# KumarRobotics/top_down_renderer

Hardware: AMD Instinct MI355X
Metric: particle-updates/sec (render+score+resample) (higher is better)
Workload: dtype f32

## Files before the change

include/tdr.h:

```cpp
#ifndef TDR_H_
#define TDR_H_

#include <stddef.h>
#include <stdint.h>

#ifdef __cplusplus
extern "C" {
#endif

#define TDR_OK 0
#define TDR_ERR_ARG (-1)
#define TDR_ERR_HIP (-2)
#define TDR_ERR_NOMEM (-3)

#define TDR_MAX_CLASSES 15
#define TDR_ST_FIELDS 7
enum { TDR_ST_INIT_X = 0, TDR_ST_INIT_Y = 1, TDR_ST_DX = 2, TDR_ST_DY = 3, TDR_ST_THETA = 4, TDR_ST_SCALE = 5,
       TDR_ST_HAVE_INIT = 6 };

typedef struct tdr_state {
  float init_x_px, init_y_px, dx_m, dy_m, theta, scale;
  uint8_t have_init;
  uint8_t pad_[3];
} tdr_state;
// ... 165 lines not shown
int tdr_config_compact(int on);
int tdr_config_shift_uniform(int mode);
float tdr_config_shift_uniform_span(float cells);
int tdr_config_ray_split(int k);
int tdr_config_cart_skip(int on);
int tdr_config_init_mfma(int on);
int tdr_config_uw_waves(int on);
int64_t tdr_shift_uniform_launches(void);

int tdr_profile_enable(int on);
int tdr_profile_score_ms(double* total_ms, int64_t* launches);
int tdr_profile_shares(double* dense_ms, double* scattered_ms, int64_t* scattered_particles);
int tdr_profile_variants(int64_t out[16]);

int64_t tdr_config_tuning(const char* name, int64_t value);
int tdr_selftest_score(void);
int tdr_k_selftest_round(const float* x, int64_t n, float limit, int32_t* out, void* stream);
int tdr_libm_variant(void);
int tdr_libm_force_variant(int variant);
int tdr_sincosf_host(const float* x, int64_t n, int variant, float* sin_out, float* cos_out);
int tdr_k_selftest_sincos(const float* x, int64_t n, float* sin_out, float* cos_out, void* stream);
int tdr_logf_host(const float* x, int64_t n, float* out);
int tdr_k_selftest_logf(const float* x, int64_t n, float* out, void* stream);
int tdr_k_selftest_atan2(const float* y, const float* x, int64_t n, float* out, void* stream);

int tdr_k_states_aos_to_soa(const tdr_state* aos, int64_t n, float* st, int64_t cap, void* stream);
int tdr_k_states_soa_to_aos(const float* st, int64_t cap, int64_t n, tdr_state* aos, void* stream);
size_t tdr_locality_tmp_ints(int64_t n, int map_rows, int map_cols);
int tdr_k_locality_order(const float* st, int64_t cap, int64_t n, int map_rows, int map_cols, int32_t* perm_out,
                         int32_t* keys_tmp, void* stream);
size_t tdr_locality_pose_tmp_ints(int64_t n);
int tdr_k_locality_order_pose(const float* st, int64_t cap, int64_t n, int map_rows, int map_cols, float theta_radius,
                              int32_t* perm_out, int32_t* keys_tmp, void* stream);

typedef struct tdr_map tdr_map;
typedef struct tdr_renderer tdr_renderer;
typedef struct tdr_filter tdr_filter;

int tdr_map_create(tdr_map** out);
void tdr_map_destroy(tdr_map* m);
int tdr_map_set(tdr_map* m, const float* class_maps, const uint8_t* class_mask, int ncls, int rows, int cols,
                float resolution, int center_x, int center_y);
int tdr_map_set_labels(tdr_map* m, const uint8_t* label_img, int img_h, int img_w, const int32_t* flatten_lut,
                       int lut_size, int ncls, float resolution, int center_x, int center_y);
int tdr_map_sample_pts_polar(tdr_map* m, int nb, int nr, float ang_res);
int tdr_map_polar_shape(const tdr_map* m, int* nb, int* nr);
int tdr_map_info(const tdr_map* m, int* ncls, int* rows, int* cols, float* resolution, int* have_map);
int tdr_map_center(const tdr_map* m, int* center_x, int* center_y);
int tdr_map_local_map(tdr_map* m, int polar, float cx, float cy, float scale_or_rot, float res, int rows, int cols,
                      float* dists_out, uint8_t* mask_out);
int tdr_map_classes_at_point(const tdr_map* m, int px, int py, uint32_t* class_bits);
int tdr_map_best_rel_pos(tdr_map* m, const float* preds, int K, float best_rel_pos[2], float* best_diff);
int tdr_map_local_geo_map(tdr_map* m, int polar, float cx, float cy, float scale_or_rot, float res, int rows, int cols,
                          float* dists_out);
int tdr_map_load_cache(tdr_map* m, const char* cache_dir, const char* map_path, int num_classes, float resolution,
                       int center_x, int center_y, int* loaded);
int tdr_map_save_cache(tdr_map* m, const char* cache_dir, const char* map_path);
int tdr_map_save_rasters(tdr_map* m, const char* dir);
int tdr_png_read_gray8_host(const char* path, uint8_t* px_out, int64_t capacity, int* w, int* h);
int tdr_png_write_gray8_host(const char* path, const uint8_t* px, int w, int h);
int tdr_map_load_rasters(tdr_map* m, const char* dir, int num_classes, float resolution, int center_x, int center_y);
#define TDR_SVG_NO_KEY 0xFFFFFFFFu
int tdr_svg_parse_host(const char* path, float size_out[2], int64_t* n_poly, int64_t* n_vert, uint32_t* keys_out,
                       int64_t* offsets_out, float* verts_out);
int tdr_map_load_polygons(tdr_map* m, const float* verts, const int64_t* poly_offsets, const int32_t* poly_class,
                          int64_t n_poly, int width, int height, int num_classes, const int32_t* exclusive, int n_excl,
// ... 79 lines not shown
```

top_down_renderer_amd/_lib.py:

```python
import ctypes as C
import os

_PKG = os.path.dirname(os.path.abspath(__file__))
SO_PATH = os.environ.get("TDR_LIB_PATH") or os.path.join(_PKG, "libtdr_hip.so")

TDR_ST_FIELDS = 7
TDR_MAX_CLASSES = 15
TDR_SVG_NO_KEY = 0xFFFFFFFF


class FilterParamsC(C.Structure):
    _fields_ = [
        ("pos_cov", C.c_float), ("theta_cov", C.c_float), ("regularization", C.c_float),
        ("init_pos_px_x", C.c_float), ("init_pos_px_y", C.c_float), ("init_pos_px_cov", C.c_float),
        ("init_pos_m_x", C.c_float), ("init_pos_m_y", C.c_float),
        ("init_pos_deg_theta", C.c_float), ("init_pos_deg_cov", C.c_float),
        ("force_on_map", C.c_int32),
        ("fixed_scale", C.c_float), ("scale_log_min", C.c_float), ("scale_log_max", C.c_float),
        ("num_classes", C.c_int32),
        ("class_weights", C.c_float * 16),
    ]


class MapDescC(C.Structure):
# ... 158 lines not shown
    "tdr_renderer_create": (_i, [_vp, C.POINTER(_vp)]),
    "tdr_renderer_destroy": (None, [_vp]),
    "tdr_renderer_render": (_i, [_vp, _i, _vp, _i, _i, _i64, _f, _f, _i, _i, _i, _vp]),
    "tdr_renderer_render_geo": (_i, [_vp, _i, _vp, _i, _i64, _i64, _f, _f, _i, _i, _vp]),
    "tdr_filter_create": (_i, [_vp, _i, C.POINTER(FilterParamsC), _u32, C.POINTER(_vp)]),
    "tdr_filter_destroy": (None, [_vp]),
    "tdr_filter_configure": (_i, [_vp, _i, _i]),
    "tdr_filter_initialize_particles": (_i, [_vp]),
    "tdr_filter_set_states": (_i, [_vp, _vp, _i64]),
    "tdr_filter_get_states": (_i, [_vp, _vp, _i64]),
    "tdr_filter_propagate": (_i, [_vp, _f, _f, _f]),
    "tdr_filter_update": (_i, [_vp, _vp, _vp, _f, _i64]),
    "tdr_filter_update_geo": (_i, [_vp, _vp, _vp, _f, _i64]),
    "tdr_filter_compute_weights": (_i, [_vp, _vp, _vp, _f]),
    "tdr_filter_get_raw_weights": (_i, [_vp, _vp, _i64]),
    "tdr_filter_get_last_dist": (_i, [_vp, _vp, _i64]),
    "tdr_filter_propagate_freeze": (_i, [_vp, _f, _f, _f, _i]),
    "tdr_filter_init_one": (_i, [_vp]),
    "tdr_filter_share_rng": (_i, [_vp, _vp]),
    "tdr_init_particle_host": (_i, [_vp, _vp, _i, _i, _i, _f, _vp, _vp]),
    "tdr_filter_get_weights": (_i, [_vp, _vp, _i64]),
    "tdr_filter_get_resample_indices": (_i, [_vp, _vp, _i64]),
    "tdr_filter_mean_cov": (_i, [_vp, _i, _vp, _vp]),
    "tdr_filter_freeze_scale": (_i, [_vp]),
    "tdr_filter_is_scale_frozen": (_i, [_vp]),
    "tdr_filter_scale": (_f, [_vp]),
    "tdr_filter_num_particles": (_i64, [_vp]),
    "tdr_filter_update_map": (_i, [_vp, _vp, _vp, _i, _i, _i, _f, _i, _i]),
    "tdr_set_error": (_i, [_i, C.c_char_p]),
    "tdr_locality_tmp_ints": (C.c_size_t, [_i64, _i, _i]),
    "tdr_locality_pose_tmp_ints": (C.c_size_t, [_i64]),
    "tdr_k_locality_order_pose": (_i, [_vp, _i64, _i64, _i, _i, _f, _vp, _vp, _vp]),
    "tdr_k_locality_order": (_i, [_vp, _i64, _i64, _i, _i, _vp, _vp, _vp]),
}

_lib = None


class TdrError(RuntimeError):
    pass


def load():
    global _lib
    if _lib is not None:
        return _lib
    if not os.path.exists(SO_PATH):
        raise TdrError(
            f"{SO_PATH} is missing: build the HIP extension first (python -m top_down_renderer_amd.build, or "
            "__graft_entry__.build()).  There is no CPU fallback.")
    L = C.CDLL(SO_PATH)
    for name, (res, args) in SIGNATURES.items():
        fn = getattr(L, name)
        fn.restype = res
        fn.argtypes = args
    _lib = L
    return L


def check(rc):
    if rc != 0:
        raise TdrError(f"libtdr_hip error {rc}: {load().tdr_last_error().decode()}")
```

top_down_renderer_amd/build.py:

```python
import os
import shutil
import subprocess
import sys
from concurrent.futures import ThreadPoolExecutor

PKG = os.path.dirname(os.path.abspath(__file__))
ROOT = os.path.dirname(PKG)
SRC = [os.path.join(PKG, "csrc", f) for f in
       ("tdr_core.hip", "tdr_map.hip", "tdr_raster.hip", "tdr_score.hip", "tdr_score_su.hip", "tdr_score_ray.hip", "tdr_score_cart.hip", "tdr_filter.hip", "tdr_rng.hip", "tdr_prefix.hip",
        "tdr_geo.hip", "tdr_cmap.hip", "tdr_active.hip", "tdr_poly.hip", "tdr_host.cpp", "tdr_comm.cpp", "tdr_gmm.cpp", "tdr_png.cpp",
        "tdr_svg.cpp")]
HDR = [os.path.join(ROOT, "include", "tdr.h")] + \
      [os.path.join(PKG, "csrc", f) for f in ("tdr_common.h", "tdr_sincosf.h", "tdr_atan2f.h", "tdr_score_su.h", "tdr_score_dev.h", "tdr_score_su_asm.h", "tdr_score_cart.h", "tdr_score_cart_asm.h", "tdr_logf.h", "tdr_mt_jump.h")]
OUT = os.path.join(PKG, "libtdr_hip.so")
OBJ_DIR = os.path.join(PKG, "_obj")
STAMP = os.path.join(PKG, "libtdr_hip.toolchain.txt")

CFLAGS = ["--offload-arch=gfx950", "-O3", "-std=c++17", "-ffp-contract=off", "-fPIC", "-I", os.path.join(ROOT, "include")]
LDFLAGS = ["--offload-arch=gfx950", "-shared", "-fPIC", "-ldl", "-lz"]
FILE_FLAGS = {"tdr_score.hip": ["-mllvm", "-amdgpu-mfma-vgpr-form"],
              "tdr_score_su.hip": ["-mllvm", "-structurizecfg-skip-uniform-regions"],
              "tdr_score_cart.hip": ["-mllvm", "-structurizecfg-skip-uniform-regions"]}


def hipcc():
    exe = shutil.which("hipcc") or "/opt/rocm/bin/hipcc"
    if not os.path.exists(exe):
        raise RuntimeError("hipcc not found: the HIP extension cannot be built (there is no CPU fallback)")
    return exe


def _obj(src):
    return os.path.join(OBJ_DIR, os.path.basename(src) + ".o")


def _stale(target, deps):
    if not os.path.exists(target):
        return True
    t = os.path.getmtime(target)
    return any(os.path.getmtime(d) > t for d in deps)


def needs_build():
    return _stale(OUT, SRC + HDR + [os.path.abspath(__file__)])


# ... 38 lines not shown
```

top_down_renderer_amd/csrc/tdr_filter.hip:

```cpp
#include <random>

#include <rocprim/device/device_radix_sort.hpp>
using TdrSortConfig = rocprim::radix_sort_config<rocprim::default_config, rocprim::merge_sort_config<512, 512, 4>, rocprim::default_config>;

#include "tdr_common.h"
#include "tdr_sincosf.h"

__device__ __forceinline__ uint32_t mulhi32(uint32_t a, uint32_t b) { return __umulhi(a, b); }
__device__ void philox4x32_10(uint32_t c[4], uint32_t k0, uint32_t k1) {
#pragma unroll
  for (int r = 0; r < 10; r++) {
    uint32_t hi0 = mulhi32(0xD2511F53u, c[0]), lo0 = 0xD2511F53u * c[0];
    uint32_t hi1 = mulhi32(0xCD9E8D57u, c[2]), lo1 = 0xCD9E8D57u * c[2];
    uint32_t n0 = hi1 ^ c[1] ^ k0, n1 = lo1, n2 = hi0 ^ c[3] ^ k1, n3 = lo0;
    c[0] = n0; c[1] = n1; c[2] = n2; c[3] = n3;
    k0 += 0x9E3779B9u; k1 += 0xBB67AE85u;
  }
}

__global__ void propagate_kernel(float* __restrict__ st, int64_t cap, int64_t n, float* __restrict__ last_dist,
                                 float tx, float ty, float omega, int scale_freeze, float pos_cov, float theta_cov,
                                 const float* __restrict__ z4, uint64_t seed, uint64_t step, int64_t index_base,
                                 int libm_fma) {
  const int64_t p = (int64_t)blockIdx.x * blockDim.x + threadIdx.x;
  if (p >= n) return;
  float z[4];
  if (z4) {
    z[0] = z4[4 * p]; z[1] = z4[4 * p + 1]; z[2] = z4[4 * p + 2]; z[3] = z4[4 * p + 3];
  } else {
    uint64_t gi = (uint64_t)(index_base + p);
    uint32_t c[4] = {(uint32_t)gi, (uint32_t)(gi >> 32), (uint32_t)step, (uint32_t)(step >> 32)};
    philox4x32_10(c, (uint32_t)seed, (uint32_t)(seed >> 32));
    float u0 = ((float)(c[0] >> 8) + 1.0f) * (1.0f / 16777216.0f), u1 = (float)(c[1] >> 8) * (1.0f / 16777216.0f);
    float u2 = ((float)(c[2] >> 8) + 1.0f) * (1.0f / 16777216.0f), u3 = (float)(c[3] >> 8) * (1.0f / 16777216.0f);
    float r0 = sqrtf(-2.0f * logf(u0)), r1 = sqrtf(-2.0f * logf(u2));
// ... 744 lines not shown
  s.dx_m = st[TDR_ST_DX * cap + p];
  s.dy_m = st[TDR_ST_DY * cap + p];
  s.theta = st[TDR_ST_THETA * cap + p];
  s.scale = st[TDR_ST_SCALE * cap + p];
  s.have_init = st[TDR_ST_HAVE_INIT * cap + p] != 0.f;
  s.pad_[0] = s.pad_[1] = s.pad_[2] = 0;
  aos[p] = s;
}
extern "C" int tdr_k_states_aos_to_soa(const tdr_state* aos, int64_t n, float* st, int64_t cap, void* stream) {
  if (!aos || !st || n < 0 || cap < n) return fail(TDR_ERR_ARG, "aos_to_soa: bad arguments");
  if (n == 0) return TDR_OK;
  hipLaunchKernelGGL(aos_to_soa_kernel, dim3((unsigned)cdiv(n, 256)), dim3(256), 0, (hipStream_t)stream, aos, n, st,
                     cap);
  LAUNCH_CHECK("aos_to_soa");
  return TDR_OK;
}
extern "C" int tdr_k_states_soa_to_aos(const float* st, int64_t cap, int64_t n, tdr_state* aos, void* stream) {
  if (!aos || !st || n < 0 || cap < n) return fail(TDR_ERR_ARG, "soa_to_aos: bad arguments");
  if (n == 0) return TDR_OK;
  hipLaunchKernelGGL(soa_to_aos_kernel, dim3((unsigned)cdiv(n, 256)), dim3(256), 0, (hipStream_t)stream, st, cap, n,
                     aos);
  LAUNCH_CHECK("soa_to_aos");
  return TDR_OK;
}

__device__ __forceinline__ uint32_t spread_bits16(uint32_t v) {
  v &= 0xFFFFu;
  v = (v | (v << 8)) & 0x00FF00FFu;
  v = (v | (v << 4)) & 0x0F0F0F0Fu;
  v = (v | (v << 2)) & 0x33333333u;
  v = (v | (v << 1)) & 0x55555555u;
  return v;
}
__global__ void loc_key_kernel(const float* __restrict__ st, int64_t cap, int64_t n, float xmax, float ymax,
                               uint32_t* __restrict__ keys, int32_t* __restrict__ vals) {
  const int64_t p = (int64_t)blockIdx.x * blockDim.x + threadIdx.x;
  if (p >= n) return;
  const float sc = st[TDR_ST_SCALE * cap + p];
  float cx = st[TDR_ST_DX * cap + p] * sc + st[TDR_ST_INIT_X * cap + p];
  float cy = st[TDR_ST_DY * cap + p] * sc + st[TDR_ST_INIT_Y * cap + p];
  if (!(cx == cx)) cx = 0.f;
  if (!(cy == cy)) cy = 0.f;
  const uint32_t hx = (uint32_t)fminf(fmaxf(cx * 2.f, 0.f), xmax);
  const uint32_t hy = (uint32_t)fminf(fmaxf(cy * 2.f, 0.f), ymax);
  keys[p] = spread_bits16(hx) | (spread_bits16(hy) << 1);
  vals[p] = (int32_t)p;
}

__device__ __forceinline__ uint64_t spread_bits21_3(uint64_t v) {
  v &= 0x1FFFFFull;
  v = (v | (v << 32)) & 0x1F00000000FFFFull;
  v = (v | (v << 16)) & 0x1F0000FF0000FFull;
  v = (v | (v << 8)) & 0x100F00F00F00F00Full;
  v = (v | (v << 4)) & 0x10C30C30C30C30C3ull;
  v = (v | (v << 2)) & 0x1249249249249249ull;
  return v;
}
__global__ void loc_key_pose_kernel(const float* __restrict__ st, int64_t cap, int64_t n, float xmax, float ymax,
                                    float theta_step, uint64_t* __restrict__ keys, int32_t* __restrict__ vals) {
  const int64_t p = (int64_t)blockIdx.x * blockDim.x + threadIdx.x;
  if (p >= n) return;
  const float sc = st[TDR_ST_SCALE * cap + p];
  float cx = st[TDR_ST_DX * cap + p] * sc + st[TDR_ST_INIT_X * cap + p];
  float cy = st[TDR_ST_DY * cap + p] * sc + st[TDR_ST_INIT_Y * cap + p];
  float th = st[TDR_ST_THETA * cap + p];
  if (!(cx == cx)) cx = 0.f;
  if (!(cy == cy)) cy = 0.f;
  if (!(fabsf(th) < 1e6f)) th = 0.f;
  th = th - 6.2831855f * floorf(th / 6.2831855f);
  const uint64_t hx = (uint64_t)fminf(fmaxf(cx * 2.f, 0.f), xmax);
  const uint64_t hy = (uint64_t)fminf(fmaxf(cy * 2.f, 0.f), ymax);
  const uint64_t ht = (uint64_t)fminf(fmaxf(th / theta_step, 0.f), 2097151.f);
  keys[p] = spread_bits21_3(hx) | (spread_bits21_3(hy) << 1) | (spread_bits21_3(ht) << 2);
  vals[p] = (int32_t)p;
}
static size_t radix_tmp_bytes64(int64_t n) {
  size_t bytes = 0;
  uint64_t* k = nullptr;
  int32_t* v = nullptr;
// ... 3 lines not shown
}
extern "C" size_t tdr_locality_pose_tmp_ints(int64_t n) {
  if (n < 1) n = 1;
  return (size_t)(5 * n + 64) + (radix_tmp_bytes64(n) + 3) / 4 + 64;
}
extern "C" int tdr_k_locality_order_pose(const float* st, int64_t cap, int64_t n, int map_rows, int map_cols,
                                         float theta_radius, int32_t* perm_out, int32_t* keys_tmp, void* stream) {
  if (!st || !perm_out || !keys_tmp || n < 0 || cap < n || map_rows < 1 || map_cols < 1 || !(theta_radius > 0.f))
    return fail(TDR_ERR_ARG, "locality_order_pose: bad arguments");
  if (map_rows > 1000000 || map_cols > 1000000) return fail(TDR_ERR_ARG, "locality_order_pose: map too large");
  if (n == 0) return TDR_OK;
  hipStream_t s = (hipStream_t)stream;
  uint64_t* keys_in = reinterpret_cast<uint64_t*>(keys_tmp);
  uint64_t* keys_out = keys_in + n;
  int32_t* vals_in = keys_tmp + 4 * n;
  void* tmp = keys_tmp + 5 * n + 64 - ((5 * n) % 64);
  size_t tmp_bytes = radix_tmp_bytes64(n);
  hipLaunchKernelGGL(loc_key_pose_kernel, dim3((unsigned)cdiv(n, 256)), dim3(256), 0, s, st, cap, n,
                     (float)(2 * map_cols - 1), (float)(2 * map_rows - 1), 0.5f / theta_radius, keys_in, vals_in);
  LAUNCH_CHECK("loc_key_pose");
  HIP_TRY(rocprim::radix_sort_pairs(tmp, tmp_bytes, keys_in, keys_out, vals_in, perm_out, (size_t)n, 0u, 63u, s, false));
  return TDR_OK;
}

static size_t radix_tmp_bytes(int64_t n) {
  size_t bytes = 0;
  uint32_t* k = nullptr;
  int32_t* v = nullptr;
  hipError_t e = rocprim::radix_sort_pairs<TdrSortConfig>(nullptr, bytes, k, k, v, v, (size_t)n, 0u, 32u, (hipStream_t)0, false);
  if (e != hipSuccess || bytes == 0) bytes = (size_t)(n + 4096) * 16;
  return bytes;
}

extern "C" size_t tdr_locality_tmp_ints(int64_t n, int map_rows, int map_cols) {
  (void)map_rows; (void)map_cols;
  if (n < 1) n = 1;
  return (size_t)(3 * n + 64) + (radix_tmp_bytes(n) + 3) / 4 + 64;
}

extern "C" int tdr_k_locality_order(const float* st, int64_t cap, int64_t n, int map_rows, int map_cols,
                                    int32_t* perm_out, int32_t* keys_tmp, void* stream) {
  if (!st || !perm_out || !keys_tmp || n < 0 || cap < n || map_rows < 1 || map_cols < 1)
    return fail(TDR_ERR_ARG, "locality_order: bad arguments");
  if (map_rows > 32767 || map_cols > 32767) return fail(TDR_ERR_ARG, "locality_order: map larger than 32767 px");
  if (n == 0) return TDR_OK;
  hipStream_t s = (hipStream_t)stream;
  uint32_t* keys_in = reinterpret_cast<uint32_t*>(keys_tmp);
  uint32_t* keys_out = keys_in + n;
  int32_t* vals_in = keys_tmp + 2 * n;
  void* tmp = keys_tmp + 3 * n + 64 - ((3 * n) % 64);
  size_t tmp_bytes = radix_tmp_bytes(n);
  hipLaunchKernelGGL(loc_key_kernel, dim3((unsigned)cdiv(n, 256)), dim3(256), 0, s, st, cap, n,
                     (float)(2 * map_cols - 1), (float)(2 * map_rows - 1), keys_in, vals_in);
  LAUNCH_CHECK("loc_key");
  unsigned bits = 2;
  while ((1u << (bits / 2)) < (unsigned)(2 * std::max(map_rows, map_cols)) && bits < 32) bits += 2;
  HIP_TRY(rocprim::radix_sort_pairs<TdrSortConfig>(tmp, tmp_bytes, keys_in, keys_out, vals_in, perm_out, (size_t)n, 0u, bits, s,
                                    false));
  return TDR_OK;
}
```

top_down_renderer_amd/csrc/tdr_score.hip:

```cpp
#include <type_traits>

#include "tdr_common.h"
#include "tdr_sincosf.h"

struct ScoreArgs {
  const float* rec;
  int rows, cols;
  float resolution;
  const float* tab;
  const float* utab;
  const float* scan_pk;
  int nb, nr;
  float res;
  const float* st;
  int64_t cap, n;
  const int32_t* order;
  const int32_t* count;
  const int32_t* slot_base;
  int use_theta_override;
  float theta_override;
  int only_uninit;
  int group, nchunks;
  int64_t npad;
  float* part;
// ... 1387 lines not shown
                                  float* __restrict__ st, int64_t cap) {
  const int64_t p = (int64_t)blockIdx.x * blockDim.x + threadIdx.x;
  if (p < n && res_flag[p] != 0.f) {
    st[TDR_ST_THETA * cap + p] = res_theta[p];
    st[TDR_ST_HAVE_INIT * cap + p] = 1.f;
  }
}
__global__ void init_fixup_kernel(const float* __restrict__ res_flag, int64_t n, float regularization,
                                  float* __restrict__ raw_w) {
  const int64_t p = (int64_t)blockIdx.x * blockDim.x + threadIdx.x;
  if (p < n && res_flag[p] == 2.f) raw_w[p] = (float)(1. / (double)(3.402823466e+38f + regularization));
}

static int g_init_mfma = 1;
static bool init_use_mfma() { return g_init_mfma != 0; }
extern "C" int tdr_config_init_mfma(int on) {
  if (on >= 0) g_init_mfma = on ? 1 : 0;
  return g_init_mfma;
}
#define TDR_CART_WAVE_MUL 2
static int64_t g_score_waves = 131072;
static int g_score_group = 0;
static int g_su_group = 0;
static int g_init_ahead = 1;
static int64_t score_wave_target() { return g_score_waves; }
extern "C" int tdr_config_prefix_head(int);
extern "C" int tdr_config_ray_block_major(int);
extern "C" int tdr_config_ray_patch(int);
extern "C" int tdr_config_ray_borrow(int);
extern "C" int tdr_config_cart_seg_rows(int);
extern "C" int tdr_config_mt_stretches(int);
extern "C" int tdr_config_su_wave_span(int);
extern "C" int tdr_config_su_lds_pad(int);
extern "C" int64_t tdr_config_tuning(const char* name, int64_t value) {
  if (!name) return -1;
  const std::string n(name);
  if (n == "score_waves") { if (value > 0) g_score_waves = value; return g_score_waves; }
  if (n == "score_group") { if (value >= 0) g_score_group = (int)value; return g_score_group; }
  if (n == "su_group") { if (value >= 0) g_su_group = (int)value; return g_su_group; }
  if (n == "init_ahead") { if (value >= 1) g_init_ahead = (int)std::min<int64_t>(value, 3); return g_init_ahead; }
  if (n == "prefix_head") return tdr_config_prefix_head((int)std::max<int64_t>(value, -1));
  if (n == "ray_borrow") return tdr_config_ray_borrow((int)std::max<int64_t>(value, -1));
  if (n == "ray_patch") return tdr_config_ray_patch((int)std::max<int64_t>(value, -1));
  if (n == "ray_block_major") return tdr_config_ray_block_major((int)std::max<int64_t>(value, -1));
  if (n == "cart_seg_rows") return tdr_config_cart_seg_rows((int)std::max<int64_t>(value, -1));
  if (n == "mt_stretches") return tdr_config_mt_stretches((int)std::max<int64_t>(value, -1));
  if (n == "su_lds_pad") return tdr_config_su_lds_pad((int)std::max<int64_t>(value, -1));
  if (n == "su_wave_span") return tdr_config_su_wave_span((int)std::max<int64_t>(value, -1));
  return -1;
}
static void choose_chunks(int64_t n, int nr, int& rpc, int& nchunks, int target_mul = 1) {
  int64_t nbatches = cdiv(std::max<int64_t>(n, 1), 64);
  int64_t want = std::max<int64_t>(1, cdiv(score_wave_target() * target_mul, nbatches));
  nchunks = (int)std::min<int64_t>(nr, want);
  rpc = (int)cdiv(nr, nchunks);
  nchunks = (int)cdiv(nr, rpc);
}

__global__ void utab_kernel(const float* __restrict__ tab, int64_t n2, float scale, float res,
                            float* __restrict__ utab) {
  const int64_t k = (int64_t)blockIdx.x * blockDim.x + threadIdx.x;
  if (k < n2) utab[k] = (tab[k] * scale) * res;
}

static int score_group_rings(int nb, int nr, int rf, int64_t n_total) {
  const int forced = g_score_group;
  const int64_t ring_bytes = std::max<int64_t>((int64_t)nb * rf * 4, 1);
  int g = (int)std::min<int64_t>(8, (32 * 1024) / ring_bytes);
  const int64_t chunks_wanted = cdiv(2048, cdiv(std::max<int64_t>(n_total, 1), 256));
  g = (int)std::min<int64_t>(g, std::max<int64_t>(1, nr / std::max<int64_t>(chunks_wanted, 1)));
  if (forced > 0) g = forced;
  g = std::max(1, std::min<int>(g, (int)((60 * 1024) / ring_bytes)));
  if (g >= TDR_SCORE_U) g -= g % TDR_SCORE_U;
  return std::max(g, 1);
}
extern "C" size_t tdr_map_rec16_bytes(int ncls, int rows, int cols) {
  if (ncls < 1 || ncls > 7 || rows < 1 || cols < 1) return 0;
  const uint64_t bytes = (uint64_t)(rows + 2) * (uint64_t)(cols + 2) * 32 + 32;
  if (bytes > 0xFFFFFFFFull || (uint64_t)(cols + 2) * 32 >= (1u << 24)) return 0;
  return (size_t)bytes;
}
// ... 733 lines not shown
```

top_down_renderer_amd/csrc/tdr_score_su.hip:

```cpp
#include <rocprim/device/device_radix_sort.hpp>

#include <atomic>

#include "tdr_score_dev.h"
#include "tdr_score_su.h"
#include "tdr_score_su_asm.h"

#define SU_CODE_FULL 0xFFu
#define SU_CODE_FULL_ALL 0xFEu
#define SU_CODE_PAD 0xFDu
#define SU_NSECT 8
#define SU_BOX_WORDS 4096

struct SuArgs {
  const uint32_t* crec;
  const uint32_t* kmask;
  int kcolw;
  unsigned kmask_off;
  const uint32_t* dict_int;
  int dict_n, ctiles_r;
  int pkcol;
  const int32_t* inexact;
  int rows, cols;
  float resolution;
  const float* tab_su;
  const uint32_t* desc;
  const float* bbox;
  const float* scan_pk;
  int nb, nr;
  float res;
  const float* st;
  int64_t cap;
  const int32_t* slots;
  const int32_t* nslots;
  int group, nchunks, ncls;
  int64_t npad;
  uint32_t* part;
// ... 768 lines not shown
    t->phase = 0;
    t->best_ms = 3.0e38f;
    t->round_best = t->best;
  }
  t->open = hipEventRecord(t->e0, s) == hipSuccess;
  t->trial_calls++;
  return kSpanCand[t->phase];
}
void tdr_su_span_end(SpanTuner* t, hipStream_t s) {
  if (g_su_span_fixed || !t || !t->open) return;
  t->open = false;
  t->pending = hipEventRecord(t->e1, s) == hipSuccess;
}
static float g_su_wave_span = 0.f;
extern "C" int tdr_config_su_wave_span(int cells) {
  if (cells >= 0) g_su_wave_span = (float)cells;
  return (int)g_su_wave_span;
}
float tdr_su_wave_span() { return g_su_wave_span; }
static int g_su_lds_pad = 0;
extern "C" int tdr_config_su_lds_pad(int bytes) {
  if (bytes >= 0) g_su_lds_pad = bytes;
  return g_su_lds_pad;
}
static std::atomic<int64_t> g_su_launches{0};
extern "C" int64_t tdr_shift_uniform_launches(void) { return g_su_launches.load(); }
bool tdr_su_shape_ok(int nb, int nr, int group, int64_t n_total) {
  if (g_su_mode == 0) return false;
  if (group % 4 != 0 || nb > 4095) return false;
  if (g_su_mode == 2) return true;
  if ((int64_t)nb * nr < 8192) return false;
  return n_total >= (int64_t)64 * nb;
}
static size_t su_sort_tmp_bytes(int64_t n) {
  size_t bytes = 0;
  uint32_t* k = nullptr;
  int32_t* v = nullptr;
  hipError_t e = rocprim::radix_sort_pairs(nullptr, bytes, k, k, v, v, (size_t)std::max<int64_t>(n, 1), 0u, 12u,
                                           (hipStream_t)0, false);
  if (e != hipSuccess || bytes == 0) bytes = (size_t)(n + 4096) * 16;
  return bytes;
}
SuWs tdr_su_ws(int nb, int nr, int group, int64_t n) {
  SuWs w;
  const int64_t nchunks = cdiv(nr, group), nbins = nchunks * nb * group;
  int64_t o = 0;
  auto take = [&](int64_t words) { const int64_t at = o; o += (words + 63) / 64 * 64; return at; };
  w.tab_su = take(2 * nbins);
  w.desc = take(4 * nbins);
  w.bbox = take(nchunks * SU_NSECT * 4);
  w.keys_in = take(n);
  w.keys_out = take(n);
  w.vals_in = take(n);
  w.vals_out = take(n);
  w.ints = take(3 * ((int64_t)nb + 1) + TDR_SU_TAIL_INTS);
  w.slots = take(su_npad(n, nb));
  w.slots2 = take(su_npad(n, nb));
  w.wave_tmp = take(2 * (su_npad(n, nb) / 64 + 1));
  w.sort_tmp = take((int64_t)((su_sort_tmp_bytes(n) + 3) / 4));
  const int64_t T = tdr_ray_padded_samples(nb, nr);
  w.ray_tab = take(2 * T);
  w.ray_desc = take((T + 1) / 2);
  w.ray_multi = take((int64_t)nb * nr);
  w.ray_rad = take(T / nb);
  w.total = o;
  return w;
}

int tdr_su_order(const SuLaunch& L, const SuWs& W, hipStream_t s, const int32_t** slots_out, const int32_t** counts_out) {
  int32_t* base = L.ws;
  uint32_t* keys_in = reinterpret_cast<uint32_t*>(base + W.keys_in);
  uint32_t* keys_out = reinterpret_cast<uint32_t*>(base + W.keys_out);
  int32_t* vals_in = base + W.vals_in;
  int32_t* vals_out = base + W.vals_out;
  int* cnt = base + W.ints;
  const int nkeys = L.nb + 1;
  int* start = cnt + nkeys;
  int* slot_start = start + nkeys;
  int* counts = slot_start + nkeys;
  int32_t* slots = base + W.slots;
  const int64_t n = L.n;
  HIP_TRY(hipMemsetAsync(cnt, 0, sizeof(int) * (size_t)(3 * nkeys + TDR_SU_TAIL_INTS), s));
  HIP_TRY(hipMemsetAsync(slots, 0xFF, sizeof(int32_t) * (size_t)L.npad, s));
  hipLaunchKernelGGL(su_key_kernel, dim3((unsigned)cdiv(n, 256)), dim3(256), sizeof(int) * (size_t)nkeys, s, L.st, L.cap, n,
                     L.perm, L.nb, L.span, keys_in, vals_in, cnt);
  LAUNCH_CHECK("su_key");
  hipLaunchKernelGGL(su_offsets_kernel, dim3(1), dim3(256), 0, s, (const int*)cnt, nkeys, start, slot_start, counts);
  LAUNCH_CHECK("su_offsets");
  unsigned bits = 1;
  while ((1u << bits) < (unsigned)nkeys) bits++;
  size_t tmp_bytes = su_sort_tmp_bytes(n);
  HIP_TRY(rocprim::radix_sort_pairs(base + W.sort_tmp, tmp_bytes, keys_in, keys_out, vals_in, vals_out, (size_t)n, 0u, bits,
                                    s, false));
  hipLaunchKernelGGL(su_scatter_kernel, dim3((unsigned)cdiv(n, 256)), dim3(256), 0, s, (const uint32_t*)keys_out,
                     (const int32_t*)vals_out, n, (const int*)start, (const int*)slot_start, slots);
  LAUNCH_CHECK("su_scatter");
  if (L.wave_span > 0.f && L.nb > 1) {
    int32_t* slots2 = base + W.slots2;
    int32_t* keep = base + W.wave_tmp;
    int32_t* moved = keep + (L.npad / 64 + 1);
    int32_t* old_counts = counts + 7;
    const int64_t nwaves = L.npad / 64;
    hipLaunchKernelGGL(su_wave_far_kernel, dim3((unsigned)cdiv(nwaves, 4)), dim3(256), 0, s, L.st, L.cap, (const int32_t*)slots,
                       (const int32_t*)counts, L.wave_span, keep, moved);
    hipLaunchKernelGGL(su_compact_offsets_kernel, dim3(1), dim3(256), 0, s, keep, moved, counts, old_counts);
    hipLaunchKernelGGL(su_compact_scatter_kernel, dim3((unsigned)cdiv(L.npad, 256)), dim3(256), 0, s, (const int32_t*)slots,
                       (const int32_t*)keep, (const int32_t*)moved, (const int32_t*)counts, (const int32_t*)old_counts, slots2);
    hipLaunchKernelGGL(su_copy_slots_kernel, dim3((unsigned)cdiv(L.npad, 256)), dim3(256), 0, s, (const int32_t*)slots2,
                       (const int32_t*)counts, slots);
    LAUNCH_CHECK("su_reroute");
  }
  *slots_out = slots;
  *counts_out = counts;
  return TDR_OK;
}
int tdr_su_prepare(const SuLaunch& L, const SuWs& W, hipStream_t s, const int32_t** slots_out, const int32_t** counts_out) {
  if (int rc = tdr_su_order(L, W, s, slots_out, counts_out)) return rc;
  int32_t* base = L.ws;
  float* tab_su = reinterpret_cast<float*>(base + W.tab_su);
  uint32_t* desc = reinterpret_cast<uint32_t*>(base + W.desc);
  const int64_t ndesc = (int64_t)L.nchunks * L.nb * L.group;
  const int lc = L.map->cwords == 1 ? 3 : (L.map->cwords == 2 ? 2 : 1);
  const int ckconst = ((L.map->rows >> lc) + 2) * 128 + 128;
  const unsigned plane_bytes = (unsigned)(tdr_cmap_plane_words(L.map->ncls, L.map->rows, L.map->cols) * 4);
  const unsigned pbase = (unsigned)(tdr_cmap_plane_offset_words(L.map->ncls, L.map->rows, L.map->cols) * 4) +
                         (unsigned)(plane_trows(L.map->rows) * 128) + 128u;
  hipLaunchKernelGGL(su_prep_kernel, dim3((unsigned)cdiv(ndesc, 256)), dim3(256), 0, s, L.tab, L.scan_pk, L.nb, L.nr, L.rf,
                     L.map->ncls, ckconst, pbase, plane_bytes, L.group, L.nchunks, L.map->dict, L.map->dict_n, tab_su, desc);
  LAUNCH_CHECK("su_prep");
  hipLaunchKernelGGL(su_bbox_kernel, dim3((unsigned)L.nchunks, SU_NSECT), dim3(256), 0, s, (const float*)tab_su, L.nb, L.nr,
                     L.group, reinterpret_cast<float*>(base + W.bbox));
  LAUNCH_CHECK("su_bbox");
  return TDR_OK;
}

int tdr_su_score(const SuLaunch& L, const SuWs& W, hipStream_t s) {
  const tdr_map_desc* map = L.map;
  int32_t* base = L.ws;
  int* nslots = base + W.ints + 3 * (L.nb + 1);
  SuArgs u;
  const int lc = map->cwords == 1 ? 3 : (map->cwords == 2 ? 2 : 1);
  u.crec = map->crec; u.dict_int = reinterpret_cast<const uint32_t*>(map->dict) + TDR_CMAP_MAX_DICT;
  u.dict_n = map->dict_n; u.ctiles_r = (map->rows >> lc) + 2;
  u.pkcol = plane_trows(map->rows) * 128 - 16;
  u.inexact = nslots + 4;
  u.rows = map->rows; u.cols = map->cols; u.resolution = map->resolution;
// ... 30 lines not shown
```

Baseline: 22.51 million.

## Replace rocprim radix sorts with custom onesweep-style radix pass for ordering

Adds a custom single-pass-per-digit radix sort kernel (9-bit digits, decoupled lookback across tiles). The locality Morton ordering now fuses key generation with histogram building and runs its own multi-pass sort for large particle counts. The SU bucket ordering becomes a single counting-sort pass that writes directly into slots when the key count fits in one digit, skipping the rocprim sort and the separate scatter kernel. The goal is to cut kernel launches and extra sort passes, at the cost of relying on spin-waiting lookback being correct and on forward progress across tiles.

After: 22.81 million (median of 6 runs). 1.3% higher.

```diff
diff --git a/include/tdr.h b/include/tdr.h
--- a/include/tdr.h
+++ b/include/tdr.h
@@ -221,6 +221,10 @@
 size_t tdr_locality_pose_tmp_ints(int64_t n);
 int tdr_k_locality_order_pose(const float* st, int64_t cap, int64_t n, int map_rows, int map_cols, float theta_radius,
                               int32_t* perm_out, int32_t* keys_tmp, void* stream);
+size_t tdr_su_order_ints(int nb, int64_t n);
+int64_t tdr_su_order_slots(int nb, int64_t n);
+int tdr_k_su_order(const float* st, int64_t cap, int64_t n, const int32_t* perm, int nb, float span, int32_t* slots_out,
+                   int32_t* counts_out, int32_t* ws, void* stream);
 
 typedef struct tdr_map tdr_map;
 typedef struct tdr_renderer tdr_renderer;
diff --git a/top_down_renderer_amd/_lib.py b/top_down_renderer_amd/_lib.py
--- a/top_down_renderer_amd/_lib.py
+++ b/top_down_renderer_amd/_lib.py
@@ -214,6 +214,9 @@
     "tdr_locality_pose_tmp_ints": (C.c_size_t, [_i64]),
     "tdr_k_locality_order_pose": (_i, [_vp, _i64, _i64, _i, _i, _f, _vp, _vp, _vp]),
     "tdr_k_locality_order": (_i, [_vp, _i64, _i64, _i, _i, _vp, _vp, _vp]),
+    "tdr_su_order_ints": (C.c_size_t, [_i, _i64]),
+    "tdr_su_order_slots": (_i64, [_i, _i64]),
+    "tdr_k_su_order": (_i, [_vp, _i64, _i64, _vp, _i, _f, _vp, _vp, _vp, _vp]),
 }
 
 _lib = None
diff --git a/top_down_renderer_amd/build.py b/top_down_renderer_amd/build.py
--- a/top_down_renderer_amd/build.py
+++ b/top_down_renderer_amd/build.py
@@ -7,11 +7,11 @@
 PKG = os.path.dirname(os.path.abspath(__file__))
 ROOT = os.path.dirname(PKG)
 SRC = [os.path.join(PKG, "csrc", f) for f in
-       ("tdr_core.hip", "tdr_map.hip", "tdr_raster.hip", "tdr_score.hip", "tdr_score_su.hip", "tdr_score_ray.hip", "tdr_score_cart.hip", "tdr_filter.hip", "tdr_rng.hip", "tdr_prefix.hip",
+       ("tdr_core.hip", "tdr_map.hip", "tdr_raster.hip", "tdr_score.hip", "tdr_score_su.hip", "tdr_score_ray.hip", "tdr_score_cart.hip", "tdr_sort.hip", "tdr_filter.hip", "tdr_rng.hip", "tdr_prefix.hip",
         "tdr_geo.hip", "tdr_cmap.hip", "tdr_active.hip", "tdr_poly.hip", "tdr_host.cpp", "tdr_comm.cpp", "tdr_gmm.cpp", "tdr_png.cpp",
         "tdr_svg.cpp")]
 HDR = [os.path.join(ROOT, "include", "tdr.h")] + \
-      [os.path.join(PKG, "csrc", f) for f in ("tdr_common.h", "tdr_sincosf.h", "tdr_atan2f.h", "tdr_score_su.h", "tdr_score_dev.h", "tdr_score_su_asm.h", "tdr_score_cart.h", "tdr_score_cart_asm.h", "tdr_logf.h", "tdr_mt_jump.h")]
+      [os.path.join(PKG, "csrc", f) for f in ("tdr_common.h", "tdr_sincosf.h", "tdr_atan2f.h", "tdr_score_su.h", "tdr_score_dev.h", "tdr_score_su_asm.h", "tdr_score_cart.h", "tdr_score_cart_asm.h", "tdr_logf.h", "tdr_mt_jump.h", "tdr_sort.h")]
 OUT = os.path.join(PKG, "libtdr_hip.so")
 OBJ_DIR = os.path.join(PKG, "_obj")
 STAMP = os.path.join(PKG, "libtdr_hip.toolchain.txt")
diff --git a/top_down_renderer_amd/csrc/tdr_filter.hip b/top_down_renderer_amd/csrc/tdr_filter.hip
--- a/top_down_renderer_amd/csrc/tdr_filter.hip
+++ b/top_down_renderer_amd/csrc/tdr_filter.hip
@@ -1,6 +1,8 @@
 #include <random>
 
 #include <rocprim/device/device_radix_sort.hpp>
+
+#include "tdr_sort.h"
 using TdrSortConfig = rocprim::radix_sort_config<rocprim::default_config, rocprim::merge_sort_config<512, 512, 4>, rocprim::default_config>;
 
 #include "tdr_common.h"
@@ -811,10 +813,7 @@
   v = (v | (v << 1)) & 0x55555555u;
   return v;
 }
-__global__ void loc_key_kernel(const float* __restrict__ st, int64_t cap, int64_t n, float xmax, float ymax,
-                               uint32_t* __restrict__ keys, int32_t* __restrict__ vals) {
-  const int64_t p = (int64_t)blockIdx.x * blockDim.x + threadIdx.x;
-  if (p >= n) return;
+__device__ __forceinline__ uint32_t loc_key_dev(const float* __restrict__ st, int64_t cap, int64_t p, float xmax, float ymax) {
   const float sc = st[TDR_ST_SCALE * cap + p];
   float cx = st[TDR_ST_DX * cap + p] * sc + st[TDR_ST_INIT_X * cap + p];
   float cy = st[TDR_ST_DY * cap + p] * sc + st[TDR_ST_INIT_Y * cap + p];
@@ -822,8 +821,32 @@
   if (!(cy == cy)) cy = 0.f;
   const uint32_t hx = (uint32_t)fminf(fmaxf(cx * 2.f, 0.f), xmax);
   const uint32_t hy = (uint32_t)fminf(fmaxf(cy * 2.f, 0.f), ymax);
-  keys[p] = spread_bits16(hx) | (spread_bits16(hy) << 1);
+  return spread_bits16(hx) | (spread_bits16(hy) << 1);
+}
+__global__ void loc_key_kernel(const float* __restrict__ st, int64_t cap, int64_t n, float xmax, float ymax,
+                               uint32_t* __restrict__ keys, int32_t* __restrict__ vals) {
+  const int64_t p = (int64_t)blockIdx.x * blockDim.x + threadIdx.x;
+  if (p >= n) return;
+  keys[p] = loc_key_dev(st, cap, p, xmax, ymax);
   vals[p] = (int32_t)p;
+}
+__global__ __launch_bounds__(RS_THREADS) void loc_key_hist_kernel(const float* __restrict__ st, int64_t cap, int64_t n, float xmax,
+                                                                  float ymax, int passes, uint32_t* __restrict__ keys,
+                                                                  uint32_t* __restrict__ hist) {
+  __shared__ uint32_t h[RS_MAX_PASSES * RS_BINS];
+  for (int k = threadIdx.x; k < passes * RS_BINS; k += RS_THREADS) h[k] = 0u;
+  __syncthreads();
+  for (int r = 0; r < RS_ITEMS; r++) {
+    const int64_t p = (int64_t)blockIdx.x * RS_TILE + r * RS_THREADS + threadIdx.x;
+    if (p < n) {
+      const uint32_t key = loc_key_dev(st, cap, p, xmax, ymax);
+      keys[p] = key;
+      for (int i = 0; i < passes; i++) atomicAdd(&h[i * RS_BINS + ((key >> (RS_BITS * i)) & (RS_BINS - 1))], 1u);
+    }
+  }
+  __syncthreads();
+  for (int k = threadIdx.x; k < passes * RS_BINS; k += RS_THREADS)
+    if (h[k]) atomicAdd(&hist[k], h[k]);
 }
 
 __device__ __forceinline__ uint64_t spread_bits21_3(uint64_t v) {
@@ -893,10 +916,24 @@
   return bytes;
 }
 
+static unsigned loc_key_bits(int map_rows, int map_cols) {
+  unsigned bits = 2;
+  while ((1u << (bits / 2)) < (unsigned)(2 * std::max(map_rows, map_cols)) && bits < 32) bits += 2;
+  return bits;
+}
+static int64_t loc_rs_words(int64_t n) { return (int64_t)RS_MAX_PASSES * (RS_BINS + rs_state_words(n)); }
+
+#define LOC_OWN_SORT_MIN 65536
+static int g_loc_sort = 1;
+extern "C" int tdr_config_loc_sort(int on) {
+  if (on >= 0) g_loc_sort = on > 2 ? 2 : on;
+  return g_loc_sort;
+}
+
 extern "C" size_t tdr_locality_tmp_ints(int64_t n, int map_rows, int map_cols) {
   (void)map_rows; (void)map_cols;
   if (n < 1) n = 1;
-  return (size_t)(3 * n + 64) + (radix_tmp_bytes(n) + 3) / 4 + 64;
+  return (size_t)(3 * n + 64) + std::max<size_t>((radix_tmp_bytes(n) + 3) / 4, (size_t)loc_rs_words(n)) + 64;
 }
 
 extern "C" int tdr_k_locality_order(const float* st, int64_t cap, int64_t n, int map_rows, int map_cols,
@@ -910,12 +947,32 @@
   uint32_t* keys_out = keys_in + n;
   int32_t* vals_in = keys_tmp + 2 * n;
   void* tmp = keys_tmp + 3 * n + 64 - ((3 * n) % 64);
+  const unsigned bits = loc_key_bits(map_rows, map_cols);
+  const float xmax = (float)(2 * map_cols - 1), ymax = (float)(2 * map_rows - 1);
+  if (g_loc_sort == 2 || (g_loc_sort == 1 && n >= LOC_OWN_SORT_MIN)) {
+    const int passes = (int)((bits + RS_BITS - 1) / RS_BITS);
+    uint32_t* hist = reinterpret_cast<uint32_t*>(tmp);
+    uint32_t* state = hist + (int64_t)RS_MAX_PASSES * RS_BINS;
+    int rc = tdr_rs_zero(hist, loc_rs_words(n), s);
+    if (rc != TDR_OK) return rc;
+    hipLaunchKernelGGL(loc_key_hist_kernel, dim3((unsigned)rs_tiles(n)), dim3(RS_THREADS), 0, s, st, cap, n, xmax, ymax, passes,
+                       keys_in, hist);
+    LAUNCH_CHECK("loc_key_hist");
+    for (int i = 0; i < passes; i++) {
+      const bool last = i == passes - 1;
+      const uint32_t* kin = i % 2 == 0 ? keys_in : keys_out;
+      uint32_t* kout = last ? nullptr : (i % 2 == 0 ? keys_out : keys_in);
+      const int32_t* vin = i == 0 ? nullptr : ((passes - i) % 2 == 0 ? perm_out : vals_in);
+      int32_t* vout = (passes - 1 - i) % 2 == 0 ? perm_out : vals_in;
+      rc = tdr_rs_pass(kin, vin, kout, vout, n, RS_BITS * i, hist + (int64_t)i * RS_BINS, nullptr, 0,
+                       state + (int64_t)i * rs_state_words(n), s);
+      if (rc != TDR_OK) return rc;
+    }
+    return TDR_OK;
+  }
   size_t tmp_bytes = radix_tmp_bytes(n);
-  hipLaunchKernelGGL(loc_key_kernel, dim3((unsigned)cdiv(n, 256)), dim3(256), 0, s, st, cap, n,
-                     (float)(2 * map_cols - 1), (float)(2 * map_rows - 1), keys_in, vals_in);
+  hipLaunchKernelGGL(loc_key_kernel, dim3((unsigned)cdiv(n, 256)), dim3(256), 0, s, st, cap, n, xmax, ymax, keys_in, vals_in);
   LAUNCH_CHECK("loc_key");
-  unsigned bits = 2;
-  while ((1u << (bits / 2)) < (unsigned)(2 * std::max(map_rows, map_cols)) && bits < 32) bits += 2;
   HIP_TRY(rocprim::radix_sort_pairs<TdrSortConfig>(tmp, tmp_bytes, keys_in, keys_out, vals_in, perm_out, (size_t)n, 0u, bits, s,
                                     false));
   return TDR_OK;
diff --git a/top_down_renderer_amd/csrc/tdr_score.hip b/top_down_renderer_amd/csrc/tdr_score.hip
--- a/top_down_renderer_amd/csrc/tdr_score.hip
+++ b/top_down_renderer_amd/csrc/tdr_score.hip
@@ -1443,6 +1443,8 @@
 extern "C" int tdr_config_mt_stretches(int);
 extern "C" int tdr_config_su_wave_span(int);
 extern "C" int tdr_config_su_lds_pad(int);
+extern "C" int tdr_config_su_count_sort(int);
+extern "C" int tdr_config_loc_sort(int);
 extern "C" int64_t tdr_config_tuning(const char* name, int64_t value) {
   if (!name) return -1;
   const std::string n(name);
@@ -1458,6 +1460,8 @@
   if (n == "mt_stretches") return tdr_config_mt_stretches((int)std::max<int64_t>(value, -1));
   if (n == "su_lds_pad") return tdr_config_su_lds_pad((int)std::max<int64_t>(value, -1));
   if (n == "su_wave_span") return tdr_config_su_wave_span((int)std::max<int64_t>(value, -1));
+  if (n == "su_count_sort") return tdr_config_su_count_sort((int)std::max<int64_t>(value, -1));
+  if (n == "loc_sort") return tdr_config_loc_sort((int)std::max<int64_t>(value, -1));
   return -1;
 }
 static void choose_chunks(int64_t n, int nr, int& rpc, int& nchunks, int target_mul = 1) {
diff --git a/top_down_renderer_amd/csrc/tdr_score_su.hip b/top_down_renderer_amd/csrc/tdr_score_su.hip
--- a/top_down_renderer_amd/csrc/tdr_score_su.hip
+++ b/top_down_renderer_amd/csrc/tdr_score_su.hip
@@ -3,6 +3,7 @@
 #include <atomic>
 
 #include "tdr_score_dev.h"
+#include "tdr_sort.h"
 #include "tdr_score_su.h"
 #include "tdr_score_su_asm.h"
 
@@ -837,6 +838,11 @@
   if ((int64_t)nb * nr < 8192) return false;
   return n_total >= (int64_t)64 * nb;
 }
+static int g_su_count_sort = 1;
+extern "C" int tdr_config_su_count_sort(int on) {
+  if (on >= 0) g_su_count_sort = on ? 1 : 0;
+  return g_su_count_sort;
+}
 static size_t su_sort_tmp_bytes(int64_t n) {
   size_t bytes = 0;
   uint32_t* k = nullptr;
@@ -858,7 +864,7 @@
   w.keys_out = take(n);
   w.vals_in = take(n);
   w.vals_out = take(n);
-  w.ints = take(3 * ((int64_t)nb + 1) + TDR_SU_TAIL_INTS);
+  w.ints = take(3 * ((int64_t)nb + 1) + TDR_SU_TAIL_INTS + rs_state_words(n));
   w.slots = take(su_npad(n, nb));
   w.slots2 = take(su_npad(n, nb));
   w.wave_tmp = take(2 * (su_npad(n, nb) / 64 + 1));
@@ -885,21 +891,27 @@
   int* counts = slot_start + nkeys;
   int32_t* slots = base + W.slots;
   const int64_t n = L.n;
-  HIP_TRY(hipMemsetAsync(cnt, 0, sizeof(int) * (size_t)(3 * nkeys + TDR_SU_TAIL_INTS), s));
+  uint32_t* rs_state = reinterpret_cast<uint32_t*>(cnt + 3 * nkeys + TDR_SU_TAIL_INTS);
+  HIP_TRY(hipMemsetAsync(cnt, 0, sizeof(int) * (size_t)(3 * nkeys + TDR_SU_TAIL_INTS + rs_state_words(n)), s));
   HIP_TRY(hipMemsetAsync(slots, 0xFF, sizeof(int32_t) * (size_t)L.npad, s));
   hipLaunchKernelGGL(su_key_kernel, dim3((unsigned)cdiv(n, 256)), dim3(256), sizeof(int) * (size_t)nkeys, s, L.st, L.cap, n,
                      L.perm, L.nb, L.span, keys_in, vals_in, cnt);
   LAUNCH_CHECK("su_key");
   hipLaunchKernelGGL(su_offsets_kernel, dim3(1), dim3(256), 0, s, (const int*)cnt, nkeys, start, slot_start, counts);
   LAUNCH_CHECK("su_offsets");
-  unsigned bits = 1;
-  while ((1u << bits) < (unsigned)nkeys) bits++;
-  size_t tmp_bytes = su_sort_tmp_bytes(n);
-  HIP_TRY(rocprim::radix_sort_pairs(base + W.sort_tmp, tmp_bytes, keys_in, keys_out, vals_in, vals_out, (size_t)n, 0u, bits,
-                                    s, false));
-  hipLaunchKernelGGL(su_scatter_kernel, dim3((unsigned)cdiv(n, 256)), dim3(256), 0, s, (const uint32_t*)keys_out,
-                     (const int32_t*)vals_out, n, (const int*)start, (const int*)slot_start, slots);
-  LAUNCH_CHECK("su_scatter");
+  if (g_su_count_sort && nkeys <= RS_BINS) {
+    const int rc = tdr_rs_pass(keys_in, vals_in, nullptr, slots, n, 0, nullptr, slot_start, nkeys, rs_state, s);
+    if (rc != TDR_OK) return rc;
+  } else {
+    unsigned bits = 1;
+    while ((1u << bits) < (unsigned)nkeys) bits++;
+    size_t tmp_bytes = su_sort_tmp_bytes(n);
+    HIP_TRY(rocprim::radix_sort_pairs(base + W.sort_tmp, tmp_bytes, keys_in, keys_out, vals_in, vals_out, (size_t)n, 0u, bits,
+                                      s, false));
+    hipLaunchKernelGGL(su_scatter_kernel, dim3((unsigned)cdiv(n, 256)), dim3(256), 0, s, (const uint32_t*)keys_out,
+                       (const int32_t*)vals_out, n, (const int*)start, (const int*)slot_start, slots);
+    LAUNCH_CHECK("su_scatter");
+  }
   if (L.wave_span > 0.f && L.nb > 1) {
     int32_t* slots2 = base + W.slots2;
     int32_t* keep = base + W.wave_tmp;
@@ -917,6 +929,29 @@
   }
   *slots_out = slots;
   *counts_out = counts;
+  return TDR_OK;
+}
+extern "C" size_t tdr_su_order_ints(int nb, int64_t n) { return (size_t)tdr_su_ws(std::max(nb, 1), 4, 4, std::max<int64_t>(n, 1)).total; }
+extern "C" int64_t tdr_su_order_slots(int nb, int64_t n) { return su_npad(std::max<int64_t>(n, 1), std::max(nb, 1)); }
+extern "C" int tdr_k_su_order(const float* st, int64_t cap, int64_t n, const int32_t* perm, int nb, float span, int32_t* slots_out,
+                              int32_t* counts_out, int32_t* ws, void* stream) {
+  if (!st || !slots_out || !counts_out || !ws || n < 1 || cap < n || nb < 1 || nb > 4095 || n > INT32_MAX / 2)
+    return fail(TDR_ERR_ARG, "su_order: bad arguments");
+  hipStream_t s = (hipStream_t)stream;
+  SuLaunch L{};
+  L.st = st;
+  L.cap = cap;
+  L.n = n;
+  L.perm = perm;
+  L.nb = nb;
+  L.span = span;
+  L.npad = su_npad(n, nb);
+  L.ws = ws;
+  const SuWs W = tdr_su_ws(nb, 4, 4, n);
+  const int32_t *slots = nullptr, *counts = nullptr;
+  if (int rc = tdr_su_order(L, W, s, &slots, &counts)) return rc;
+  HIP_TRY(hipMemcpyAsync(slots_out, slots, sizeof(int32_t) * (size_t)L.npad, hipMemcpyDeviceToDevice, s));
+  HIP_TRY(hipMemcpyAsync(counts_out, counts, sizeof(int32_t) * 3, hipMemcpyDeviceToDevice, s));
   return TDR_OK;
 }
 int tdr_su_prepare(const SuLaunch& L, const SuWs& W, hipStream_t s, const int32_t** slots_out, const int32_t** counts_out) {
diff --git a/top_down_renderer_amd/csrc/tdr_sort.h b/top_down_renderer_amd/csrc/tdr_sort.h
--- /dev/null
+++ b/top_down_renderer_amd/csrc/tdr_sort.h
@@ -0,0 +1,19 @@
+#ifndef TDR_SORT_H_
+#define TDR_SORT_H_
+#include "tdr_common.h"
+
+#define RS_BITS 9
+#define RS_BINS (1 << RS_BITS)
+#define RS_THREADS 256
+#define RS_ITEMS 8
+#define RS_TILE (RS_THREADS * RS_ITEMS)
+#define RS_MAX_PASSES 4
+#define RS_STATE_HEAD 64
+
+static inline int64_t rs_tiles(int64_t n) { return cdiv(std::max<int64_t>(n, 1), RS_TILE); }
+static inline int64_t rs_state_words(int64_t n) { return RS_STATE_HEAD + rs_tiles(n) * RS_BINS; }
+
+int tdr_rs_pass(const uint32_t* keys_in, const int32_t* vals_in, uint32_t* keys_out, int32_t* vals_out, int64_t n, int shift,
+                const uint32_t* ghist, const int32_t* gstart, int nstart, uint32_t* state, hipStream_t s);
+int tdr_rs_zero(uint32_t* words, int64_t nwords, hipStream_t s);
+#endif
diff --git a/top_down_renderer_amd/csrc/tdr_sort.hip b/top_down_renderer_amd/csrc/tdr_sort.hip
--- /dev/null
+++ b/top_down_renderer_amd/csrc/tdr_sort.hip
@@ -0,0 +1,162 @@
+#include "tdr_sort.h"
+
+#define RS_FLAG_AGG (1u << 30)
+#define RS_FLAG_INC (2u << 30)
+#define RS_COUNT_MASK ((1u << 30) - 1u)
+#define RS_LOOKBACK 16
+
+__global__ __launch_bounds__(RS_THREADS) void rs_zero_kernel(uint32_t* __restrict__ p, int64_t n) {
+  for (int64_t i = (int64_t)blockIdx.x * blockDim.x + threadIdx.x; i < n; i += (int64_t)gridDim.x * blockDim.x) p[i] = 0u;
+}
+
+__global__ __launch_bounds__(RS_THREADS) void rs_pass_kernel(const uint32_t* __restrict__ keys_in, const int32_t* __restrict__ vals_in,
+                                                             uint32_t* __restrict__ keys_out, int32_t* __restrict__ vals_out,
+                                                             int64_t n, int shift, const uint32_t* __restrict__ ghist,
+                                                             const int32_t* __restrict__ gstart, int nstart,
+                                                             uint32_t* __restrict__ state) {
+  __shared__ uint32_t s_base[RS_BINS];
+  __shared__ uint32_t s_cnt[RS_THREADS / 64][RS_BINS];
+  __shared__ uint32_t s_scan[RS_THREADS];
+  __shared__ int64_t s_tile;
+  const int tid = threadIdx.x, lane = tid & 63, w = tid >> 6;
+  if (tid == 0) s_tile = (int64_t)atomicAdd(state, 1u);
+  for (int d = tid; d < RS_BINS; d += RS_THREADS) s_cnt[0][d] = 0u;
+  __syncthreads();
+  const int64_t tile = s_tile, base = tile * RS_TILE;
+  uint32_t key[RS_ITEMS], dig[RS_ITEMS];
+  int32_t val[RS_ITEMS];
+#pragma unroll
+  for (int r = 0; r < RS_ITEMS; r++) {
+    const int64_t i = base + r * RS_THREADS + tid;
+    dig[r] = RS_BINS;
+    key[r] = 0u;
+    val[r] = 0;
+    if (i < n) {
+      key[r] = keys_in[i];
+      dig[r] = (key[r] >> shift) & (RS_BINS - 1);
+      val[r] = vals_in ? vals_in[i] : (int32_t)i;
+      atomicAdd(&s_cnt[0][dig[r]], 1u);
+    }
+  }
+  __syncthreads();
+  uint32_t* flags = state + RS_STATE_HEAD;
+  uint32_t cnt[RS_BINS / RS_THREADS], start[RS_BINS / RS_THREADS];
+#pragma unroll
+  for (int j = 0; j < RS_BINS / RS_THREADS; j++) {
+    const int d = tid + j * RS_THREADS;
+    cnt[j] = s_cnt[0][d];
+    __hip_atomic_store(&flags[tile * RS_BINS + d], (tile == 0 ? RS_FLAG_INC : RS_FLAG_AGG) | cnt[j], __ATOMIC_RELAXED,
+                       __HIP_MEMORY_SCOPE_AGENT);
+  }
+  if (gstart) {
+#pragma unroll
+    for (int j = 0; j < RS_BINS / RS_THREADS; j++) {
+      const int d = tid + j * RS_THREADS;
+      start[j] = d < nstart ? (uint32_t)gstart[d] : 0u;
+    }
+  } else {
+    const uint32_t h0 = ghist[2 * tid], h1 = ghist[2 * tid + 1];
+    s_scan[tid] = h0 + h1;
+    __syncthreads();
+    for (int o = 1; o < RS_THREADS; o <<= 1) {
+      const uint32_t v = tid >= o ? s_scan[tid - o] : 0u;
+      __syncthreads();
+      s_scan[tid] += v;
+      __syncthreads();
+    }
+    const uint32_t ex = s_scan[tid] - h0 - h1;
+    s_base[2 * tid] = ex;
+    s_base[2 * tid + 1] = ex + h0;
+    __syncthreads();
+#pragma unroll
+    for (int j = 0; j < RS_BINS / RS_THREADS; j++) start[j] = s_base[tid + j * RS_THREADS];
+  }
+#pragma unroll
+  for (int j = 0; j < RS_BINS / RS_THREADS; j++) {
+    const int d = tid + j * RS_THREADS;
+    uint32_t before = 0u;
+    if (tile > 0) {
+      for (int64_t hi = tile - 1; hi >= 0;) {
+        uint32_t f[RS_LOOKBACK];
+#pragma unroll
+        for (int q = 0; q < RS_LOOKBACK; q++)
+          f[q] = __hip_atomic_load(&flags[(hi - q >= 0 ? hi - q : 0) * RS_BINS + d], __ATOMIC_RELAXED, __HIP_MEMORY_SCOPE_AGENT);
+#pragma unroll
+        for (int q = 0; q < RS_LOOKBACK; q++)
+          if (hi - q < 0) f[q] = RS_FLAG_INC;
+        uint32_t sum = 0u;
+        bool ready = true, done = false;
+#pragma unroll
+        for (int q = 0; q < RS_LOOKBACK; q++) {
+          if (done || !ready) continue;
+          if ((f[q] >> 30) == 0u) { ready = false; continue; }
+          sum += f[q] & RS_COUNT_MASK;
+          done = (f[q] >> 30) == 2u;
+        }
+        if (!ready) continue;
+        before += sum;
+        if (done) break;
+        hi -= RS_LOOKBACK;
+      }
+      __hip_atomic_store(&flags[tile * RS_BINS + d], RS_FLAG_INC | (before + cnt[j]), __ATOMIC_RELAXED,
+                         __HIP_MEMORY_SCOPE_AGENT);
+    }
+    start[j] += before;
+  }
+  __syncthreads();
+#pragma unroll
+  for (int j = 0; j < RS_BINS / RS_THREADS; j++) s_base[tid + j * RS_THREADS] = start[j];
+  const uint64_t below = (1ull << lane) - 1ull;
+#pragma unroll
+  for (int r = 0; r < RS_ITEMS; r++) {
+    for (int k = tid; k < (RS_THREADS / 64) * RS_BINS; k += RS_THREADS) (&s_cnt[0][0])[k] = 0u;
+    __syncthreads();
+    const uint32_t d = dig[r];
+    const bool ok = d < RS_BINS;
+    uint64_t same = __ballot(ok);
+#pragma unroll
+    for (int b = 0; b < RS_BITS; b++) {
+      const bool bit = (d >> b) & 1u;
+      const uint64_t m = __ballot(bit);
+      same &= bit ? m : ~m;
+    }
+    const uint32_t rank = (uint32_t)__popcll(same & below);
+    if (ok && rank == 0u) s_cnt[w][d] = (uint32_t)__popcll(same);
+    __syncthreads();
+    if (ok) {
+      uint32_t at = s_base[d] + rank;
+      for (int v = 0; v < w; v++) at += s_cnt[v][d];
+      if (keys_out) keys_out[at] = key[r];
+      vals_out[at] = val[r];
+    }
+    __syncthreads();
+#pragma unroll
+    for (int j = 0; j < RS_BINS / RS_THREADS; j++) {
+      const int e = tid + j * RS_THREADS;
+      uint32_t add = 0u;
+#pragma unroll
+      for (int v = 0; v < RS_THREADS / 64; v++) add += s_cnt[v][e];
+      s_base[e] += add;
+    }
+    __syncthreads();
+  }
+}
+
+int tdr_rs_pass(const uint32_t* keys_in, const int32_t* vals_in, uint32_t* keys_out, int32_t* vals_out, int64_t n, int shift,
+                const uint32_t* ghist, const int32_t* gstart, int nstart, uint32_t* state, hipStream_t s) {
+  if (n < 0 || n > (int64_t)RS_COUNT_MASK || !keys_in || !vals_out || !state || (!ghist && !gstart) || shift < 0 || shift > 31)
+    return fail(TDR_ERR_ARG, "radix pass: bad arguments");
+  if (n == 0) return TDR_OK;
+  hipLaunchKernelGGL(rs_pass_kernel, dim3((unsigned)rs_tiles(n)), dim3(RS_THREADS), 0, s, keys_in, vals_in, keys_out, vals_out, n,
+                     shift, ghist, gstart, nstart, state);
+  LAUNCH_CHECK("rs_pass");
+  return TDR_OK;
+}
+
+int tdr_rs_zero(uint32_t* words, int64_t nwords, hipStream_t s) {
+  if (nwords <= 0) return TDR_OK;
+  const int64_t blocks = std::min<int64_t>(cdiv(nwords, RS_THREADS), 1024);
+  hipLaunchKernelGGL(rs_zero_kernel, dim3((unsigned)blocks), dim3(RS_THREADS), 0, s, words, nwords);
+  LAUNCH_CHECK("rs_zero");
+  return TDR_OK;
+}
```
